# koide3/small_gicp

Measured on AMD Instinct MI355X. Metric: GICP iterations/sec (1M<->1M pts), higher is better.
Workload: dtype f32; 1 GPU; C3: GICP, per-point covariances k=20, 1000000 target <-> 1000000 source points, max_corr_dist 1.0 m; parallelism=single GPU

## Files before the change

include/small_gicp_amd_debug.h:

```cpp
#ifndef SMALL_GICP_AMD_DEBUG_H
#define SMALL_GICP_AMD_DEBUG_H

#include "small_gicp_amd.h"

#ifdef __cplusplus
extern "C" {
#endif

int sga_problem_set_search_stats(sga_context* ctx, sga_problem* pb, int enabled);
int sga_problem_get_search_stats(sga_context* ctx, const sga_problem* pb, int* leaves_per_point);
int sga_problem_get_sorted_points(sga_context* ctx, const sga_problem* pb, float* xyzw);
int sga_problem_get_last_plan(const sga_problem* pb, int out[8]);
int sga_problem_get_grid_stats(const sga_problem* pb, uint64_t out[6]);
void sga_set_grid_mode(int mode, long long min_points);
void sga_set_knn_wave_max(long long max_points);
int sga_index_spacing(const sga_index* index, double* spacing);
int sga_debug_kd_tree(sga_context* ctx, const sga_index* index, int* depth, float* nodes, float* xyzw);
int sga_debug_index_bbox(const sga_index* index, float lo[3], float hi[3]);
int sga_debug_forest_launches(unsigned long long* launches);
int sga_debug_voxelgrid_plan(const sga_cloud* cloud, double leaf, int out[9]);
int sga_debug_set_voxelgrid_epoch(sga_context* ctx, unsigned epoch);
int sga_debug_timer_start(sga_context* ctx);
int sga_debug_timer_stop(sga_context* ctx, double* ms);
#define SGA_FRAME_CHECK_DOUBLES 32
void sga_debug_shard_frame_pack(const double origin[3], double out[SGA_FRAME_CHECK_DOUBLES]);
int sga_debug_shard_frame_agree(const double sum[SGA_FRAME_CHECK_DOUBLES]);
int sga_debug_kd_trips(unsigned long long* out16);
int sga_debug_kd_wave_times(unsigned long long* out, int waves);

#ifdef __cplusplus
}
#endif
#endif
```

small_gicp_amd/_lib.py:

```python
import ctypes as C
import os
import sys

_HERE = os.path.dirname(os.path.abspath(__file__))
LIB_PATH = os.environ.get("SGA_LIB_PATH") or os.path.join(_HERE, "lib", "libsmall_gicp_amd.so")

SGA_OK = 0
ICP, PLANE_ICP, GICP = 0, 1, 2
FLAT_NORMALS, FLAT_COVS = 1, 2
ROBUST_NONE, ROBUST_HUBER, ROBUST_CAUCHY = 0, 1, 2
LEVENBERG_MARQUARDT, GAUSS_NEWTON = 0, 1
MATH_FP32, MATH_FP64 = 0, 1
ACCUM_DOUBLES = 30


class SgaError(RuntimeError):
    pass


class FactorParams(C.Structure):
    _fields_ = [("factor_kind", C.c_int), ("robust_kind", C.c_int), ("robust_c", C.c_double), ("max_dist_sq", C.c_double), ("math_mode", C.c_int)]


class RegistrationSettingC(C.Structure):
# ... 121 lines not shown
    ("sga_problem_get_sorted_points", C.c_int, [C.c_void_p, C.c_void_p, C.c_void_p]),
    ("sga_problem_get_grid_stats", C.c_int, [C.c_void_p, C.POINTER(C.c_uint64)]),
    ("sga_problem_get_last_plan", C.c_int, [C.c_void_p, C.POINTER(C.c_int)]),
    ("sga_set_grid_mode", None, [C.c_int, C.c_longlong]),
    ("sga_host_alloc", C.c_int, [C.c_size_t, C.POINTER(C.c_void_p)]),
    ("sga_host_free", C.c_int, [C.c_void_p]),
    ("sga_index_spacing", C.c_int, [C.c_void_p, C.POINTER(C.c_double)]),
    ("sga_set_knn_wave_max", None, [C.c_longlong]),
    ("sga_debug_kd_tree", C.c_int, [C.c_void_p, C.c_void_p, C.POINTER(C.c_int), C.c_void_p, C.c_void_p]),
    ("sga_debug_voxelgrid_plan", C.c_int, [C.c_void_p, C.c_double, C.POINTER(C.c_int)]),
    ("sga_debug_set_voxelgrid_epoch", C.c_int, [C.c_void_p, C.c_uint]),
    ("sga_debug_timer_start", C.c_int, [C.c_void_p]),
    ("sga_debug_timer_stop", C.c_int, [C.c_void_p, C.POINTER(C.c_double)]),
    ("sga_debug_shard_frame_pack", None, [C.POINTER(C.c_double), C.POINTER(C.c_double)]),
    ("sga_debug_shard_frame_agree", C.c_int, [C.POINTER(C.c_double)]),
    ("sga_debug_kd_trips", C.c_int, [C.c_void_p]),
    ("sga_debug_kd_wave_times", C.c_int, [C.c_void_p, C.c_int]),
    ("sga_set_search_mode", None, [C.c_int, C.c_int, C.c_int]),
    ("sga_get_warm_limit", C.c_double, []),
    ("sga_problem_get_pass_stats", C.c_int, [_vp, _vp, C.POINTER(C.c_uint64), C.POINTER(C.c_uint64), C.POINTER(C.c_uint64)]),
    ("sga_registration_setting_default", None, [C.POINTER(RegistrationSettingC)]),
    ("sga_align", C.c_int, [_vp, _vp, _vp, _dp, C.POINTER(RegistrationSettingC), C.POINTER(ResultC)]),
    ("sga_align_problem", C.c_int, [_vp, _vp, _dp, C.POINTER(RegistrationSettingC), C.POINTER(ResultC)]),
    ("sga_multi_create", C.c_int, [C.POINTER(C.c_int), C.c_int, _pvp]),
    ("sga_multi_destroy", C.c_int, [_vp]),
    ("sga_multi_num_devices", C.c_int, [_vp]),
    ("sga_multi_set_target_f64", C.c_int, [_vp, _dp, _dp, _dp, C.c_size_t]),
    ("sga_multi_set_target_f32", C.c_int, [_vp, _fp, _fp, _fp, C.c_size_t]),
    ("sga_multi_set_source_f32", C.c_int, [_vp, _fp, _fp, _fp, C.c_size_t, _dp]),
    ("sga_multi_set_target_f32_origin", C.c_int, [_vp, _fp, _fp, _fp, C.c_size_t, _dp]),
# ... 46 lines not shown
```

small_gicp_amd/api.py:

```python
import ctypes as C

import numpy as np

from . import _lib
from ._lib import GICP, ICP, PLANE_ICP, FactorParams, RegistrationSettingC, ResultC, check, load

_FACTOR_BY_NAME = {"ICP": ICP, "PLANE_ICP": PLANE_ICP, "GICP": GICP, "VGICP": GICP}


def _fp(a):
    return None if a is None else a.ctypes.data_as(C.POINTER(C.c_float))


def _dp(a):
    return None if a is None else a.ctypes.data_as(C.POINTER(C.c_double))


def _T16(T):
    T = np.eye(4) if T is None else np.asarray(T, dtype=np.float64).reshape(4, 4)
    return np.ascontiguousarray(T.T).reshape(16)


class Context:

# ... 759 lines not shown
        return RegistrationResult(res)

    def search_stats(self, enable=None):
        if enable is not None:
            check(load().sga_problem_set_search_stats(self.ctx.h, self.h, 1 if enable else 0))
            return None
        out = np.zeros(len(self.source), dtype=np.int32)
        check(load().sga_problem_get_search_stats(self.ctx.h, self.h, out.ctypes.data_as(C.c_void_p)))
        return out

    def sorted_points(self):
        out = np.zeros((len(self.source), 4), dtype=np.float32)
        check(load().sga_problem_get_sorted_points(self.ctx.h, self.h, out.ctypes.data_as(C.c_void_p)))
        return out

    def pass_stats(self):
        c, w, f = C.c_uint64(), C.c_uint64(), C.c_uint64()
        check(load().sga_problem_get_pass_stats(self.ctx.h, self.h, C.byref(c), C.byref(w), C.byref(f)))
        g = (C.c_uint64 * 6)()
        check(load().sga_problem_get_grid_stats(self.h, g))
        return {"cold_passes": c.value, "warm_passes": w.value, "walked_points": f.value, "grid_passes": g[0], "grid_open": g[1], "grid_rings": g[2], "grid_cell_m": g[3] * 1e-6,
                "adj_queries": g[4], "adj_unsettled": g[5]}


def _T16s(Ts, count):
    if Ts is None:
        Ts = [None] * count
    if len(Ts) != count:
        raise ValueError(f"{len(Ts)} poses for {count} pairs")
    return np.ascontiguousarray(np.stack([_T16(T) for T in Ts]).reshape(count, 16)) if count else np.zeros((0, 16))


class BatchProblem:

    def __init__(self, problems):
        self.problems = list(problems)
        self.ctx = self.problems[0].ctx if self.problems else default_context()
# ... 333 lines not shown
```

small_gicp_amd/csrc/common.hpp:

```cpp
#pragma once
#include <hip/hip_runtime.h>

#include <atomic>
#include <cstdarg>
#include <cstdint>
#include <cstdio>
#include <cstdlib>
#include <cstring>
#include <string>
#include <vector>

#include "../../include/small_gicp_amd.h"
#include "../../include/small_gicp_amd_debug.h"

namespace sga {

void set_error(const char* fmt, ...);
int fail(int code, const char* fmt, ...);

#define SGA_HIP(expr)                                                                                             \
  do {                                                                                                            \
    hipError_t _e = (expr);                                                                                       \
    if (_e != hipSuccess) return ::sga::fail(SGA_ERR_HIP, "%s:%d %s -> %s", __FILE__, __LINE__, #expr, hipGetErrorString(_e)); \
  } while (0)
// ... 219 lines not shown
  bool frame_checked = false;
  bool has_normals = false, has_covs = false;
  sga::DevBuf<float4> pts;
  sga::DevBuf<sga::Cov8> cov;
  const float4* pts_view = nullptr;
  const sga::Cov8* cov_view = nullptr;
  const float4* src_pts() const { return pts_view ? pts_view : pts.p; }
  const sga::Cov8* src_cov() const { return cov_view ? cov_view : cov.p; }
  sga::DevBuf<int> corr;
  sga::DevBuf<int> hint;
  sga::DevBuf<int> hint2;
  sga::DevBuf<float> rex;
  sga::DevBuf<int> dbg_leaves;
  sga::DevBuf<uint32_t> walked;
  bool state_fresh = false;
  double T_prev[16] = {0};
  bool prev_valid = false;
  int prev_math = 0;
  int lin_factor = -1;
  double lin_T[16] = {0};
  bool maha_valid = false;
  int last_math = 0;
  float bbox_lo[3] = {0, 0, 0}, bbox_hi[3] = {0, 0, 0};
  uint64_t cold_passes = 0, warm_passes = 0;
  uint64_t grid_passes = 0;
  sga::DevBuf<uint32_t> grid_stats;
  bool grid_stats_pending = false;
  uint64_t grid_open_total = 0, grid_ring_total = 0;
  double grid_open_frac = 0.0;
  sga::DevBuf<uint32_t> tile_cost, tile_order;
// ... 15 lines not shown
```

small_gicp_amd/csrc/linearize.hip:

```cpp
#include <algorithm>
#include <chrono>
#include <thread>
#include <type_traits>
#include <utility>

#include "batch.hpp"
#include "common.hpp"
#include "device_math.hpp"
#include "uniform.hpp"
#include "cell_grid.hpp"
#include "kd_search.hpp"
#include "projective.hpp"
#include "voxel_hash.hpp"

void sga_profile_collect_pending(sga_context* ctx);

namespace sga {

int comm_allreduce_sum(sga_context* ctx, double* d_buf, size_t count);
template <typename Real>
int grid_search_pass(sga_context* ctx, const sga_index* idx, const float4* src_pts, int n, const Rigid<Real>& T, float reach2, int* nn, int* nn2, float* rex, uint32_t* stats);
int grid_rings_for(const sga_index* idx, double reach);

#ifndef SGA_SPACING_REF
// ... 126 lines not shown

template <typename Real>
struct NNParams {
  const float4* __restrict__ src_pts;
  int n;
  KdView kd;
  Rigid<Real> T;
  float bound2;
  float within2;
  float slack_min, slack_max;
  float cert_pad;
  int* __restrict__ nn;
  int* __restrict__ nn2;
  float* __restrict__ rex;
  int check;
  Rigid<Real> T_prev;
  uint32_t* __restrict__ walked;
  const uint32_t* __restrict__ tile_order;
  uint32_t* __restrict__ tile_cost;
  int* __restrict__ leaves;
  double inv_leaf;
  int chunk_tiles;
  int fast;
  GridView grid;
  int grid_walk;
};

__device__ __forceinline__ float certify(float rex, float moved, bool has_neighbour, float d2_new, float within2, float pad) {
  const float lim = rex - moved * 1.000001f;
  const float lim_d = lim - moved * pad;
// ... 9 lines not shown
  if (!exact) {
    const KdBestFast f = kd_nearest_fast<BLOCK>(p.kd, fx, fy, fz, p.bound2, seed, kd_stack, tid, slack);
    nb = f.best;
    exact = f.ambiguous;
  }
  if (exact) nb = kd_nearest<BLOCK>(p.kd, fx, fy, fz, p.bound2, seed, kd_stack, tid, slack);
  p.nn[i] = nb.idx;
  p.nn2[i] = nb.idx2;
  p.rex[i] = rex_from_r2(nb.r2);
  if (p.leaves != nullptr) p.leaves[i] = nb.leaves;
  return nb.idx;
}

template <typename Real, int BLOCK, bool CHECK>
__device__ __forceinline__ int search_lane(const NNParams<Real>& p, int tile, int i, const float4& ps, float fx, float fy, float fz, uint32_t* __restrict__ kd_stack) {
  int seed = p.nn[i];
  float slack = 0.f;
  if constexpr (CHECK) {
    Real ox, oy, oz;
    transform_point<Real>(p.T_prev, ps.x, ps.y, ps.z, ox, oy, oz);
    const float moved = sqrtf(kd_dist2(static_cast<float>(ox), static_cast<float>(oy), static_cast<float>(oz), fx, fy, fz));
    const int cand2 = p.nn2[i];
    float d1 = INFINITY, d2 = INFINITY;
    if (seed >= 0) {
      const float4 c = p.kd.pts[seed];
      d1 = kd_dist2(c.x, c.y, c.z, fx, fy, fz);
    }
    if (cand2 >= 0) {
      const float4 c = p.kd.pts[cand2];
      d2 = kd_dist2(c.x, c.y, c.z, fx, fy, fz);
    }
// ... 98 lines not shown
  uint32_t node = 1;
  int depth = 0, sp = 0;
  KdState s = kd_state(p.bound2, 0.f);

  for (;;) {
    while (tile < tile_end && q_count <= kQueueCap - 64) {
      const int i = tile * 64 + lane;
      bool need = i < p.n;
      float fx = 0.f, fy = 0.f, fz = 0.f, slack = 0.f;
      int seed = -1, cand2 = -1;
      if (need) {
        const float4 ps = p.src_pts[i];
        Real x, y, z;
        transform_point<Real>(p.T, ps.x, ps.y, ps.z, x, y, z);
        fx = static_cast<float>(x), fy = static_cast<float>(y), fz = static_cast<float>(z);
        seed = p.nn[i];
        cand2 = p.nn2[i];
        if constexpr (CHECK) {
          Real ox, oy, oz;
          transform_point<Real>(p.T_prev, ps.x, ps.y, ps.z, ox, oy, oz);
          const float moved = sqrtf(kd_dist2(static_cast<float>(ox), static_cast<float>(oy), static_cast<float>(oz), fx, fy, fz));
          float d1 = INFINITY, d2 = INFINITY;
          if (seed >= 0) {
            const float4 c = p.kd.pts[seed];
            d1 = kd_dist2(c.x, c.y, c.z, fx, fy, fz);
          }
          if (cand2 >= 0) {
            const float4 c = p.kd.pts[cand2];
            d2 = kd_dist2(c.x, c.y, c.z, fx, fy, fz);
          }
          const bool swap = cand2 >= 0 && (d2 < d1 || (d2 == d1 && cand2 < seed));
          const int best = swap ? cand2 : seed;
// ... 876 lines not shown
    acc += wave_sum_f64(static_cast<double>(e));
  }
  if (lane == 0) sh_e[wave] = acc;
  __syncthreads();
  if (threadIdx.x == 0) {
    double s = 0.0;
    for (int w = 0; w < kTile / 64; w++) s += sh_e[w];
    if (p.tail.enabled)
      __hip_atomic_store(&p.partials[blockIdx.x], s, __ATOMIC_RELAXED, __HIP_MEMORY_SCOPE_AGENT);
    else
      p.partials[blockIdx.x] = s;
  }
  if (p.tail.enabled) fused_tail(p.tail, p.partials, gridDim.x, 1, 1);
}

constexpr int kReduceGroups = 64;

constexpr int kReduceSlices = 8;
__global__ __launch_bounds__(kReduceSlices * kCols) void reduce_rows_kernel(
  const double* __restrict__ partials, int nrows, int ncols, int row_stride, double* __restrict__ stage, unsigned* __restrict__ ticket, double* __restrict__ out, int out_n, double* __restrict__ host,
  unsigned long long seq, int derive, const uint32_t* __restrict__ stats) {
  __shared__ double sh[kReduceSlices][kCols];
  __shared__ unsigned sh_ticket;
  const int c = threadIdx.x & (kCols - 1), s = threadIdx.x / kCols;
  const int G = gridDim.x;
  double a0 = 0.0, a1 = 0.0, a2 = 0.0, a3 = 0.0;
  if (c < ncols) {
    const int step = G * kReduceSlices;
    int r = blockIdx.x + G * s;
    for (; r + 3 * step < nrows; r += 4 * step) {
      const double v0 = partials[static_cast<size_t>(r) * row_stride + c], v1 = partials[static_cast<size_t>(r + step) * row_stride + c];
      const double v2 = partials[static_cast<size_t>(r + 2 * step) * row_stride + c], v3 = partials[static_cast<size_t>(r + 3 * step) * row_stride + c];
      a0 += v0, a1 += v1, a2 += v2, a3 += v3;
    }
    for (; r < nrows; r += step) a0 += partials[static_cast<size_t>(r) * row_stride + c];
  }
  sh[s][c] = (a0 + a1) + (a2 + a3);
  __syncthreads();
  auto fold = [&]() {
    if (threadIdx.x < kCols) {
      double t = 0.0;
#pragma unroll
      for (int k = 0; k < kReduceSlices; k++) t += sh[k][threadIdx.x];
      sh[0][threadIdx.x] = t;
    }
    __syncthreads();
  };
  fold();
  if (G > 1) {
    if (threadIdx.x < kCols) __hip_atomic_store(&stage[blockIdx.x * kCols + threadIdx.x], sh[0][threadIdx.x], __ATOMIC_RELAXED, __HIP_MEMORY_SCOPE_AGENT);
    asm volatile("s_waitcnt vmcnt(0)" ::: "memory");
    __syncthreads();
// ... 27 lines not shown
  if (G > 1 && threadIdx.x == 0) __hip_atomic_store(ticket, 0u, __ATOMIC_RELAXED, __HIP_MEMORY_SCOPE_AGENT);
  if (host != nullptr) {
    __threadfence_system();
    __syncthreads();
    if (threadIdx.x == 0) __hip_atomic_store(reinterpret_cast<unsigned long long*>(host + kSeqWord), seq, __ATOMIC_RELEASE, __HIP_MEMORY_SCOPE_SYSTEM);
  }
}

__global__ __launch_bounds__(kReduceSlices * kCols) void batch_reduce_rows_kernel(const BatchPair* __restrict__ pairs, unsigned* __restrict__ ticket, double* __restrict__ host, double* __restrict__ seq_word, unsigned long long seq) {
  __shared__ double sh[kReduceSlices][kCols];
  __shared__ unsigned sh_ticket;
  const BatchPair* d = uniform_const(pairs + blockIdx.x);
  const double* __restrict__ partials = d->p.partials;
  const int nrows = d->ntiles, out_row = d->pair;
  const int c = threadIdx.x & (kCols - 1), s = threadIdx.x / kCols;
  double a0 = 0.0, a1 = 0.0, a2 = 0.0, a3 = 0.0;
  if (c < kModelCols) {
    constexpr int step = kReduceSlices;
    int r = s;
    for (; r + 3 * step < nrows; r += 4 * step) {
      const double v0 = partials[static_cast<size_t>(r) * kRow + c], v1 = partials[static_cast<size_t>(r + step) * kRow + c];
      const double v2 = partials[static_cast<size_t>(r + 2 * step) * kRow + c], v3 = partials[static_cast<size_t>(r + 3 * step) * kRow + c];
      a0 += v0, a1 += v1, a2 += v2, a3 += v3;
    }
    for (; r < nrows; r += step) a0 += partials[static_cast<size_t>(r) * kRow + c];
  }
  sh[s][c] = (a0 + a1) + (a2 + a3);
  __syncthreads();
  if (threadIdx.x < kCols) {
    double t = 0.0;
#pragma unroll
    for (int k = 0; k < kReduceSlices; k++) t += sh[k][threadIdx.x];
    sh[0][threadIdx.x] = t;
  }
  __syncthreads();
  if (threadIdx.x < kRow) {
    const int cc = threadIdx.x;
    const double t = is_derived_col(cc) ? derived_entry(cc, sh[0]) : sh[0][cc];
    host[static_cast<size_t>(out_row) * kRow + cc] = cc < kModelCols ? t : 0.0;
  }
  __threadfence_system();
  __syncthreads();
  if (threadIdx.x == 0) sh_ticket = __hip_atomic_fetch_add(ticket, 1u, __ATOMIC_ACQ_REL, __HIP_MEMORY_SCOPE_AGENT);
  __syncthreads();
  if (sh_ticket != gridDim.x - 1) return;
  if (threadIdx.x == 0) {
    __hip_atomic_store(ticket, 0u, __ATOMIC_RELAXED, __HIP_MEMORY_SCOPE_AGENT);
    __threadfence_system();
    __hip_atomic_store(reinterpret_cast<unsigned long long*>(seq_word), seq, __ATOMIC_RELEASE, __HIP_MEMORY_SCOPE_SYSTEM);
  }
}

__global__ __launch_bounds__(1024) void tile_order_kernel(const uint32_t* __restrict__ cost, uint32_t* __restrict__ order, int num_tiles) {
  __shared__ uint32_t hist[64], start[64];
  const int per_xcd = num_tiles >> 3;
  const int x = blockIdx.x, first = x * per_xcd;
  if (threadIdx.x < 64) hist[threadIdx.x] = 0u;
  __syncthreads();
  for (int k = threadIdx.x; k < per_xcd; k += blockDim.x) atomicAdd(&hist[63u - min(63u, cost[first + k] >> 8)], 1u);
  __syncthreads();
  if (threadIdx.x == 0) {
    uint32_t acc = 0u;
    for (int b = 0; b < 64; b++) {
      start[b] = acc;
      acc += hist[b];
    }
  }
  __syncthreads();
  for (int k = threadIdx.x; k < per_xcd; k += blockDim.x) {
    const uint32_t pos = atomicAdd(&start[63u - min(63u, cost[first + k] >> 8)], 1u);
    order[first + pos] = static_cast<uint32_t>(first + k);
  }
  if (x == 0)
    for (int t = 8 * per_xcd + threadIdx.x; t < num_tiles; t += blockDim.x) order[t] = static_cast<uint32_t>(t);
}

static size_t partial_rows(size_t n) { return std::max<size_t>(kMaxBlocks, (n + 63) / 64); }

static int reduce_groups(int nrows) { return nrows > 256 ? std::min(kReduceGroups, std::max(8, nrows / 128)) : 1; }

static void launch_reduce(sga_context* ctx, const double* partials, int nrows, int ncols, int row_stride, double* stage, double* out, int out_n, double* host, unsigned long long seq, bool derive = false, const uint32_t* stats = nullptr) {
  const int groups = reduce_groups(nrows);
  hipLaunchKernelGGL(reduce_rows_kernel, dim3(groups), dim3(kReduceSlices * kCols), 0, ctx->stream, partials, nrows, ncols, row_stride, stage, ctx->d_ticket.p, out, out_n, host, seq, derive ? 1 : 0, stats);
}

template <typename T>
static T env_or(const char* name, T d) {
  const char* s = getenv(name);
  return s == nullptr ? d : std::is_floating_point_v<T> ? static_cast<T>(atof(s)) : static_cast<T>(atoll(s));
}

constexpr int kLinPts = 4;
constexpr int kLinPtsMin = 750000;
constexpr int kLinPtsMinF64 = 131072;

static double g_warm_delta = env_or("SGA_WARM_DELTA", 0.1);

static int g_search_queue = env_or("SGA_SEARCH_QUEUE", 2);
// ... 231 lines not shown
  q.kd = p.kd;
  q.T = p.T;
  q.within2 = p.bound2;
  q.slack_min = static_cast<float>(kSlackMin * unit), q.slack_max = static_cast<float>(kSlackMax * unit);
  q.cert_pad = std::max(g_cert_pad, 0.f);
  q.bound2 = p.bound2 * (1.f + kSearchMargin) * (1.f + kSearchMargin);
  q.nn = pb->hint.p, q.nn2 = pb->hint2.p, q.rex = pb->rex.p, q.walked = pb->walked.p;
  q.fast = g_fast_scan;
  q.leaves = pb->dbg_leaves.n >= pb->n ? pb->dbg_leaves.p : nullptr;

  const PassPlan plan = plan_pass<Real>(ctx, pb, q, displacement, unit, host_rejector);
  p.num_tiles = factor_tiles(p.n, plan.pts);
  const int blocks = grid_blocks(p.num_tiles);
  p.tail = FusedTail{plan.tail ? 1 : 0, ctx->d_ticket.p, d_out30, out_n, host, seq};
  q.check = plan.warm ? 1 : 0;
  if (plan.warm) q.T_prev = rigid_from_colmajor<Real>(pb->T_prev);
  if (plan.grid) {
    q.grid_walk = g_grid_walk;
    q.grid = make_grid_view(idx);
  }
  q.chunk_tiles = plan.chunk_tiles;

  const bool timed = ctx->profiling && (ctx->lin_seq++ % ctx->profile_period) == 0;
  if (timed) {
    sga_profile_collect_pending(ctx);
    (void)hipEventRecord(ctx->ev0, ctx->stream);
    ctx->pending_warm = plan.warm;
  }
  int rows = p.n > 0 ? blocks : 0;
  const bool first_pass = !pb->prev_valid;
  if (!voxel) pb->prev_valid = false;
  pb->state_fresh = false;
  if (plan.route != Route::kFactors) {
    if (q.leaves != nullptr) SGA_HIP(hipMemsetAsync(q.leaves, 0, pb->n * sizeof(int), ctx->stream));
    if (plan.grid && (first_pass || (plan.route != Route::kGrid && !plan.warm))) pb->grid_open_frac = 0.0;
    pb->order_tiles = 0;
    const size_t words = static_cast<size_t>(p.kd.depth);
    const dim3 sgrid((p.n + kSearchBlock - 1) / kSearchBlock), sblock(kSearchBlock);
    switch (plan.route) {
      case Route::kGrid:
        if (pb->grid_stats.n < 4) {
          SGA_TRY(pb->grid_stats.alloc(4));
          SGA_HIP(hipMemsetAsync(pb->grid_stats.p, 0, 4 * sizeof(uint32_t), ctx->stream));
        }
        SGA_TRY(grid_search_pass<Real>(ctx, idx, pb->src_pts(), p.n, p.T, q.bound2, pb->hint.p, pb->hint2.p, pb->rex.p, pb->grid_stats.p));
        pb->grid_passes++;
        break;
      case Route::kCertify:
        if constexpr (sizeof(Real) == 4) {
          p.cert_nn = q.nn, p.cert_nn2 = q.nn2, p.cert_rex = q.rex, p.cert_walked = q.walked;
          p.T_prev = q.T_prev, p.cert_within2 = q.within2, p.cert_pad = q.cert_pad;
          p.cert_slack_min = q.slack_min, p.cert_slack_max = q.slack_max;
          const size_t lds = std::max<size_t>(words, 1) * 64 * sizeof(uint32_t) * (kTile / 64);
          with_factor(fp->factor_kind, [&](auto f) { hipLaunchKernelGGL((certify_linearize_kernel<Real, decltype(f)::value, 1>), dim3(blocks), dim3(kTile), lds, ctx->stream, p, q); });
        }
        break;
      case Route::kFusedLane:
        if constexpr (sizeof(Real) == 4) {
// ... 68 lines not shown
    }
  }
  if (p.n > 0 && !plan.fused()) {
    with_factor(fp->factor_kind, [&](auto f) {
      constexpr int F = decltype(f)::value;
      if (flat)
        launch_linearize<Real, F, 2>(ctx->stream, p, blocks, plan.pts);
      else if (proj) {
        hipLaunchKernelGGL((projective_linearize_kernel<Real, F, 1>), dim3(blocks), dim3(kTile), 0, ctx->stream, p, make_proj_view(idx));
      } else if (voxel) {
        if constexpr (F != SGA_PLANE_ICP) launch_linearize<Real, F, 1>(ctx->stream, p, blocks, plan.pts);
      } else
        launch_linearize<Real, F, 0>(ctx->stream, p, blocks, plan.pts);
    });
  }
  if (!plan.tail) launch_reduce(ctx, pb->partials.p, rows, ncols, kRow, pb->partials.p + partial_rows(pb->n) * kRow, d_out30, out_n, host, seq, true, plan.route == Route::kGrid ? pb->grid_stats.p : nullptr);
  pb->grid_stats_pending = plan.route == Route::kGrid && !plan.tail && out_n > kStatsCol + 1;
  {
    const int lp[8] = {static_cast<int>(plan.route), plan.warm, plan.grid, plan.pts, plan.tail, plan.chunk_tiles, plan.tail ? 0 : rows, plan.tail ? 0 : reduce_groups(rows)};
    std::copy(lp, lp + 8, pb->last_plan);
  }
  if (timed) {
    (void)hipEventRecord(ctx->ev1, ctx->stream);
    ctx->pending |= 1;
  }
  if (plan.order_record) {
    hipLaunchKernelGGL(tile_order_kernel, dim3(8), dim3(1024), 0, ctx->stream, pb->tile_cost.p, pb->tile_order.p, rows);
    pb->order_tiles = static_cast<unsigned>(rows);
    pb->order_stream = ctx->stream;
  }
  SGA_HIP(hipGetLastError());
  pb->last_math = math;
  pb->lin_factor = fp->factor_kind;
  memcpy(pb->lin_T, T, sizeof(pb->lin_T));
  pb->maha_valid = p.store_maha != 0;
  if (!voxel) {
    memcpy(pb->T_prev, T, sizeof(pb->T_prev));
    pb->prev_valid = true;
    pb->prev_math = math;
    if (plan.warm)
      pb->warm_passes++;
    else
      pb->cold_passes++;
  }
  return SGA_OK;
}

template <typename Real>
__global__ void recompute_maha_kernel(const Cov8* __restrict__ src_cov, const Cov8* __restrict__ tgt_cov, const int* __restrict__ corr, int n, Rigid<Real> T, Real* __restrict__ maha) {
  const int i = blockIdx.x * blockDim.x + threadIdx.x;
  if (i >= n) return;
  const int j = corr[i];
  if (j < 0) return;
  const Sym3<Real> Cs = load_sym<Real>(src_cov, i);
// ... 418 lines not shown
    const double* Tp = problem_pose(pb, T + 16 * k, Td);
    if (Tp != Td) memcpy(Td, Tp, 16 * sizeof(double));
    BatchPair d{};
    d.p = factor_params<float>(pb, fp, Td, false);
    d.p.kd = make_kd_view(idx);
    d.p.partials = pb->partials.p;
    d.q.src_pts = pb->src_pts();
    d.q.n = d.p.n;
    d.q.kd = d.p.kd;
    d.q.T = d.p.T;
    d.q.within2 = d.p.bound2;
    d.q.bound2 = d.p.bound2 * (1.f + kSearchMargin) * (1.f + kSearchMargin);
    d.q.nn = pb->hint.p, d.q.nn2 = pb->hint2.p, d.q.rex = pb->rex.p, d.q.walked = pb->walked.p;
    d.q.fast = g_fast_scan;
    d.ntiles = bt->tiles[k];
    d.seedless = seedless ? 1 : 0;
    d.pair = k;
    prefix[a] = blocks;
    blocks += (d.ntiles + 7) / 8 * 8;
    pairs[a] = d;
  }
  prefix[order.size()] = blocks;
  const int nactive = static_cast<int>(order.size());
  const unsigned long long seq = ++bt->seq;
  SGA_HIP(hipMemcpyAsync(bt->d_round.p, bt->h_round, batch_round_bytes(count), hipMemcpyHostToDevice, ctx->stream));
  const int* d_prefix = reinterpret_cast<const int*>(bt->d_round.p);
  const BatchPair* d_pairs = reinterpret_cast<const BatchPair*>(bt->d_round.p + batch_pairs_offset(count));
  for (int k : order) {
    sga_problem* pb = bt->problems[k];
    pb->prev_valid = false;
    pb->model_valid = false;
// ... 11 lines not shown
  if (rc != SGA_OK) {
    (void)hipMemsetAsync(bt->ticket.p, 0, sizeof(unsigned), ctx->stream);
    return rc;
  }
  for (size_t a = 0; a < order.size(); a++) {
    const int k = order[a];
    sga_problem* pb = bt->problems[k];
    const double* Td = &Tdev[16 * a];
    pb->last_math = SGA_MATH_FP32;
    pb->lin_factor = fp->factor_kind;
    memcpy(pb->lin_T, Td, sizeof(pb->lin_T));
    pb->maha_valid = false;
    memcpy(pb->T_prev, Td, sizeof(pb->T_prev));
    pb->prev_valid = true;
    pb->prev_math = SGA_MATH_FP32;
    pb->cold_passes++;
    pb->grid_stats_pending = false;
    const int lp[8] = {static_cast<int>(Route::kFusedLane), 0, 0, 1, 0, 0, bt->tiles[k], 1};
    std::copy(lp, lp + 8, pb->last_plan);
    memcpy(pb->model, bt->h_out + static_cast<size_t>(k) * kRow, sizeof(pb->model));
    memcpy(pb->model_T, Td, sizeof(pb->model_T));
    pb->model_valid = true;
  }
  return SGA_OK;
}
}

extern "C" {

int sga_linearize(sga_context* ctx, sga_problem* pb, const sga_factor_params* fp, const double T[16], double H[36], double b[6], double* e, uint64_t* num_inliers) {
// ... 101 lines not shown
  if (enabled) return pb->dbg_leaves.alloc(pb->n);
  pb->dbg_leaves.release();
  return SGA_OK;
}
int sga_problem_get_sorted_points(sga_context* ctx, const sga_problem* pb, float* xyzw) {
  if (!ctx || !pb || !xyzw) return fail(SGA_ERR_INVALID, "null argument");
  if (pb->n == 0) return SGA_OK;
  SGA_ENTER(ctx);
  SGA_HIP(hipMemcpyAsync(xyzw, pb->src_pts(), pb->n * sizeof(float4), hipMemcpyDeviceToHost, ctx->stream));
  SGA_HIP(hipStreamSynchronize(ctx->stream));
  return SGA_OK;
}
int sga_problem_get_last_plan(const sga_problem* pb, int out[8]) {
  if (!pb || !out) return fail(SGA_ERR_INVALID, "null argument");
  std::copy(pb->last_plan, pb->last_plan + 8, out);
  return SGA_OK;
}
int sga_problem_get_search_stats(sga_context* ctx, const sga_problem* pb, int* leaves_per_point) {
  if (!ctx || !pb || !leaves_per_point) return fail(SGA_ERR_INVALID, "null argument");
  if (pb->dbg_leaves.n < pb->n) return fail(SGA_ERR_INVALID, "search statistics are not enabled");
  SGA_ENTER(ctx);
  SGA_HIP(hipMemcpyAsync(leaves_per_point, pb->dbg_leaves.p, pb->n * sizeof(int), hipMemcpyDeviceToHost, ctx->stream));
  SGA_HIP(hipStreamSynchronize(ctx->stream));
  return SGA_OK;
}

#ifdef SGA_KD_TRIPS
int sga_debug_kd_trips(unsigned long long* out16) {
  unsigned long long zero[16] = {0};
  if (hipMemcpyFromSymbol(out16, HIP_SYMBOL(g_kd_trips), sizeof(zero)) != hipSuccess) return SGA_ERR_HIP;
// ... 19 lines not shown
#define SGA_PRELOAD_FACTOR(F)                                        \
  SGA_PRELOAD(search_linearize_kernel<float, F, false>);            \
  SGA_PRELOAD(search_linearize_kernel<float, F, true>);             \
  SGA_PRELOAD(nn_search_queue_kernel<float, true, F>);              \
  SGA_PRELOAD(certify_linearize_kernel<float, F, 1>);               \
  SGA_PRELOAD(linearize_kernel<float, F, 0, kLinPts>);              \
  SGA_PRELOAD(linearize_kernel<float, F, 0, 1>);                   \
  SGA_PRELOAD(batch_search_linearize_kernel<F>)
  SGA_PRELOAD_FACTOR(SGA_GICP);
  SGA_PRELOAD_FACTOR(SGA_PLANE_ICP);
  SGA_PRELOAD_FACTOR(SGA_ICP);
  SGA_PRELOAD(linearize_kernel<float, SGA_GICP, 1, kLinPts>);
  SGA_PRELOAD(linearize_kernel<float, SGA_GICP, 1, 1>);
  SGA_PRELOAD(reduce_rows_kernel);
  SGA_PRELOAD(batch_reduce_rows_kernel);
  SGA_PRELOAD(tile_order_kernel);
  SGA_PRELOAD(publish_kernel);
  SGA_PRELOAD(error_kernel<float, SGA_GICP>);
#undef SGA_PRELOAD_FACTOR
#undef SGA_PRELOAD
  (void)hipGetLastError();
}
}

extern "C" {

void sga_set_grid_mode(int mode, long long min_points) {
  if (mode >= 0) sga::g_grid_mode = mode;
  if (min_points >= 0) sga::g_grid_min_points = min_points;
}

// ... 8 lines not shown
```

small_gicp_amd/csrc/optimizer.hip:

```cpp
#include <cmath>
#include <cstdio>

#include "batch.hpp"
#include "common.hpp"

namespace sga {

struct M4 {
  double a[16];
};

static M4 mul(const M4& A, const M4& B) {
  M4 C;
  for (int c = 0; c < 4; c++)
    for (int r = 0; r < 4; r++) {
      double s = 0;
      for (int k = 0; k < 4; k++) s += A.a[4 * k + r] * B.a[4 * c + k];
      C.a[4 * c + r] = s;
    }
  return C;
}

static M4 se3_exp(const double d[6]) {
  const double wx = d[0], wy = d[1], wz = d[2];
// ... 352 lines not shown
  const M4 m = se3_exp(twist);
  memcpy(T, m.a, sizeof(m.a));
}

int sga_optimize(const sga_registration_setting* setting, const double init_T[16], sga_linearize_fn linearize, sga_error_fn error, void* user, sga_result* out) {
  if (!setting || !init_T || !linearize || !out) return fail(SGA_ERR_INVALID, "null argument");
  if (setting->optimizer == SGA_LEVENBERG_MARQUARDT && !error) return fail(SGA_ERR_INVALID, "LM needs an error callback");
  return optimize_impl(*setting, init_T, linearize, error, user, out);
}

int sga_align_problem(sga_context* ctx, sga_problem* problem, const double init_T[16], const sga_registration_setting* setting, sga_result* out) {
  if (!ctx || !problem || !setting || !out) return fail(SGA_ERR_INVALID, "null argument");
  static const double I16[16] = {1, 0, 0, 0, 0, 1, 0, 0, 0, 0, 1, 0, 0, 0, 0, 1};
  if (problem->target->n <= 10) std::fprintf(stderr, "warning: target point cloud is too small. |target|=%zu\n", problem->target->n);
  if (problem->n <= 10) std::fprintf(stderr, "warning: source point cloud is too small. |source|=%zu\n", problem->n);
  if (!problem->state_fresh) {
    SGA_HIP(hipSetDevice(ctx->device));
    if (problem->n > 0) SGA_HIP(hipMemsetAsync(problem->hint.p, 0xff, problem->n * sizeof(int), ctx->stream));
    if (problem->n > 0 && problem->hint2.n >= problem->n) SGA_HIP(hipMemsetAsync(problem->hint2.p, 0xff, problem->n * sizeof(int), ctx->stream));
  }
  problem->prev_valid = false;
  GpuReduction g{ctx, problem, &setting->factor};
  return optimize_impl(*setting, init_T ? init_T : I16, gpu_linearize, gpu_error, &g, out);
}

int sga_optimize_batch(const sga_registration_setting* setting, size_t count, const double* init_T, sga_batch_linearize_fn linearize, sga_batch_error_fn error, void* user, sga_result* out) {
  if (!setting || !linearize) return fail(SGA_ERR_INVALID, "null argument");
  if (setting->optimizer == SGA_LEVENBERG_MARQUARDT && !error) return fail(SGA_ERR_INVALID, "LM needs an error callback");
  if (count == 0) return SGA_OK;
  if (!out) return fail(SGA_ERR_INVALID, "null argument");
  return optimize_batch_impl(*setting, count, init_T, linearize, error, user, out);
}

int sga_align_batch(sga_context* ctx, sga_batch* batch, const double* init_T, const sga_registration_setting* setting, sga_result* out) {
  if (!setting) return fail(SGA_ERR_INVALID, "null argument");
// ... 25 lines not shown
```

Measured before the change: 8908 iterations/s.

## Fold tile-order sort into reduce kernel and replace hint memsets with seedless flag

The separate tile_order_kernel launch is removed and its work is done by eight extra blocks appended to the reduce_rows grid. The per-align hipMemsetAsync calls that reset the nn/nn2 hint arrays are replaced by a hints_void flag, which makes the first cold pass ignore the stale seeds. Both changes cut kernel/memset launches per pass and per align, at the cost of a more complex reduce kernel and extra state tracking. Debug counters and introspection APIs are also added.

```diff
diff --git a/include/small_gicp_amd_debug.h b/include/small_gicp_amd_debug.h
--- a/include/small_gicp_amd_debug.h
+++ b/include/small_gicp_amd_debug.h
@@ -25,6 +25,10 @@
 #define SGA_FRAME_CHECK_DOUBLES 32
 void sga_debug_shard_frame_pack(const double origin[3], double out[SGA_FRAME_CHECK_DOUBLES]);
 int sga_debug_shard_frame_agree(const double sum[SGA_FRAME_CHECK_DOUBLES]);
+int sga_debug_reduce_rows(sga_context* ctx, const double* rows, int nrows, int derive, int groups, int kind, double out[96]);
+int sga_problem_get_search_state(sga_context* ctx, const sga_problem* pb, int* nn, int* nn2, float* rex);
+int sga_problem_get_tile_order(sga_context* ctx, const sga_problem* pb, unsigned* cost, unsigned* order, size_t capacity, size_t* tiles);
+int sga_debug_pass_launches(unsigned long long out[3]);
 int sga_debug_kd_trips(unsigned long long* out16);
 int sga_debug_kd_wave_times(unsigned long long* out, int waves);
 
diff --git a/small_gicp_amd/_lib.py b/small_gicp_amd/_lib.py
--- a/small_gicp_amd/_lib.py
+++ b/small_gicp_amd/_lib.py
@@ -159,6 +159,10 @@
     ("sga_debug_timer_stop", C.c_int, [C.c_void_p, C.POINTER(C.c_double)]),
     ("sga_debug_shard_frame_pack", None, [C.POINTER(C.c_double), C.POINTER(C.c_double)]),
     ("sga_debug_shard_frame_agree", C.c_int, [C.POINTER(C.c_double)]),
+    ("sga_debug_reduce_rows", C.c_int, [C.c_void_p, C.c_void_p, C.c_int, C.c_int, C.c_int, C.c_int, C.POINTER(C.c_double)]),
+    ("sga_problem_get_search_state", C.c_int, [C.c_void_p, C.c_void_p, C.c_void_p, C.c_void_p, C.c_void_p]),
+    ("sga_problem_get_tile_order", C.c_int, [C.c_void_p, C.c_void_p, C.c_void_p, C.c_void_p, C.c_size_t, C.POINTER(C.c_size_t)]),
+    ("sga_debug_pass_launches", C.c_int, [C.POINTER(C.c_ulonglong)]),
     ("sga_debug_kd_trips", C.c_int, [C.c_void_p]),
     ("sga_debug_kd_wave_times", C.c_int, [C.c_void_p, C.c_int]),
     ("sga_set_search_mode", None, [C.c_int, C.c_int, C.c_int]),
diff --git a/small_gicp_amd/api.py b/small_gicp_amd/api.py
--- a/small_gicp_amd/api.py
+++ b/small_gicp_amd/api.py
@@ -797,6 +797,20 @@
         check(load().sga_problem_get_sorted_points(self.ctx.h, self.h, out.ctypes.data_as(C.c_void_p)))
         return out
 
+    def search_state(self):
+        n = len(self.source)
+        nn, nn2, rex = np.zeros(n, np.int32), np.zeros(n, np.int32), np.zeros(n, np.float32)
+        check(load().sga_problem_get_search_state(self.ctx.h, self.h, nn.ctypes.data_as(C.c_void_p), nn2.ctypes.data_as(C.c_void_p), rex.ctypes.data_as(C.c_void_p)))
+        return nn, nn2, rex
+
+    def tile_order(self):
+        tiles = C.c_size_t()
+        check(load().sga_problem_get_tile_order(self.ctx.h, self.h, None, None, 0, C.byref(tiles)))
+        cost, order = np.zeros(tiles.value, np.uint32), np.zeros(tiles.value, np.uint32)
+        if tiles.value:
+            check(load().sga_problem_get_tile_order(self.ctx.h, self.h, cost.ctypes.data_as(C.c_void_p), order.ctypes.data_as(C.c_void_p), tiles.value, C.byref(tiles)))
+        return cost, order
+
     def pass_stats(self):
         c, w, f = C.c_uint64(), C.c_uint64(), C.c_uint64()
         check(load().sga_problem_get_pass_stats(self.ctx.h, self.h, C.byref(c), C.byref(w), C.byref(f)))
@@ -804,6 +818,20 @@
         check(load().sga_problem_get_grid_stats(self.h, g))
         return {"cold_passes": c.value, "warm_passes": w.value, "walked_points": f.value, "grid_passes": g[0], "grid_open": g[1], "grid_rings": g[2], "grid_cell_m": g[3] * 1e-6,
                 "adj_queries": g[4], "adj_unsettled": g[5]}
+
+
+def debug_reduce_rows(rows, derive=False, groups=0, batch=False, ctx=None):
+    rows = np.ascontiguousarray(rows, dtype=np.float64).reshape(-1, 96)
+    out = np.zeros(96)
+    c = ctx or default_context()
+    check(load().sga_debug_reduce_rows(c.h, rows.ctypes.data_as(C.c_void_p), rows.shape[0], 1 if derive else 0, int(groups), 1 if batch else 0, _dp(out)))
+    return out
+
+
+def debug_pass_launches():
+    v = (C.c_ulonglong * 3)()
+    check(load().sga_debug_pass_launches(v))
+    return {"reduce": v[0], "reduce_with_sort": v[1], "fills": v[2]}
 
 
 def _T16s(Ts, count):
diff --git a/small_gicp_amd/csrc/common.hpp b/small_gicp_amd/csrc/common.hpp
--- a/small_gicp_amd/csrc/common.hpp
+++ b/small_gicp_amd/csrc/common.hpp
@@ -257,6 +257,7 @@
   sga::DevBuf<int> dbg_leaves;
   sga::DevBuf<uint32_t> walked;
   bool state_fresh = false;
+  bool hints_void = false;
   double T_prev[16] = {0};
   bool prev_valid = false;
   int prev_math = 0;
diff --git a/small_gicp_amd/csrc/linearize.hip b/small_gicp_amd/csrc/linearize.hip
--- a/small_gicp_amd/csrc/linearize.hip
+++ b/small_gicp_amd/csrc/linearize.hip
@@ -1,4 +1,5 @@
 #include <algorithm>
+#include <atomic>
 #include <chrono>
 #include <thread>
 #include <type_traits>
@@ -164,6 +165,7 @@
   int* __restrict__ nn2;
   float* __restrict__ rex;
   int check;
+  int seedless;
   Rigid<Real> T_prev;
   uint32_t* __restrict__ walked;
   const uint32_t* __restrict__ tile_order;
@@ -203,7 +205,7 @@
 
 template <typename Real, int BLOCK, bool CHECK>
 __device__ __forceinline__ int search_lane(const NNParams<Real>& p, int tile, int i, const float4& ps, float fx, float fy, float fz, uint32_t* __restrict__ kd_stack) {
-  int seed = p.nn[i];
+  int seed = p.seedless ? -1 : p.nn[i];
   float slack = 0.f;
   if constexpr (CHECK) {
     Real ox, oy, oz;
@@ -332,8 +334,10 @@
         Real x, y, z;
         transform_point<Real>(p.T, ps.x, ps.y, ps.z, x, y, z);
         fx = static_cast<float>(x), fy = static_cast<float>(y), fz = static_cast<float>(z);
-        seed = p.nn[i];
-        cand2 = p.nn2[i];
+        if (!p.seedless) {
+          seed = p.nn[i];
+          cand2 = p.nn2[i];
+        }
         if constexpr (CHECK) {
           Real ox, oy, oz;
           transform_point<Real>(p.T_prev, ps.x, ps.y, ps.z, ox, oy, oz);
@@ -1240,28 +1244,58 @@
   if (p.tail.enabled) fused_tail(p.tail, p.partials, gridDim.x, 1, 1);
 }
 
+__device__ __forceinline__ void tile_order_share(const uint32_t* __restrict__ cost, uint32_t* __restrict__ order, int num_tiles, int x) {
+  __shared__ uint32_t hist[64], start[64];
+  const int per_xcd = num_tiles >> 3;
+  const int first = x * per_xcd;
+  if (threadIdx.x < 64) hist[threadIdx.x] = 0u;
+  __syncthreads();
+  for (int k = threadIdx.x; k < per_xcd; k += blockDim.x) atomicAdd(&hist[63u - min(63u, cost[first + k] >> 8)], 1u);
+  __syncthreads();
+  if (threadIdx.x == 0) {
+    uint32_t acc = 0u;
+    for (int b = 0; b < 64; b++) {
+      start[b] = acc;
+      acc += hist[b];
+    }
+  }
+  __syncthreads();
+  for (int k = threadIdx.x; k < per_xcd; k += blockDim.x) {
+    const uint32_t pos = atomicAdd(&start[63u - min(63u, cost[first + k] >> 8)], 1u);
+    order[first + pos] = static_cast<uint32_t>(first + k);
+  }
+  if (x == 0)
+    for (int t = 8 * per_xcd + threadIdx.x; t < num_tiles; t += blockDim.x) order[t] = static_cast<uint32_t>(t);
+}
+
 constexpr int kReduceGroups = 64;
+static std::atomic<unsigned long long> g_pass_launches[3];
 
 constexpr int kReduceSlices = 8;
+
+__device__ __forceinline__ double sum_rows_chains(const double* __restrict__ partials, int r0, int step, int nrows, int row_stride, int c) {
+  double a0 = 0.0, a1 = 0.0, a2 = 0.0, a3 = 0.0;
+  int r = r0;
+  for (; r + 3 * step < nrows; r += 4 * step) {
+    const double v0 = partials[static_cast<size_t>(r) * row_stride + c], v1 = partials[static_cast<size_t>(r + step) * row_stride + c];
+    const double v2 = partials[static_cast<size_t>(r + 2 * step) * row_stride + c], v3 = partials[static_cast<size_t>(r + 3 * step) * row_stride + c];
+    a0 += v0, a1 += v1, a2 += v2, a3 += v3;
+  }
+  for (; r < nrows; r += step) a0 += partials[static_cast<size_t>(r) * row_stride + c];
+  return (a0 + a1) + (a2 + a3);
+}
+
 __global__ __launch_bounds__(kReduceSlices * kCols) void reduce_rows_kernel(
-  const double* __restrict__ partials, int nrows, int ncols, int row_stride, double* __restrict__ stage, unsigned* __restrict__ ticket, double* __restrict__ out, int out_n, double* __restrict__ host,
-  unsigned long long seq, int derive, const uint32_t* __restrict__ stats) {
+  const double* __restrict__ partials, int nrows, int ncols, int row_stride, int G, double* __restrict__ stage, unsigned* __restrict__ ticket, double* __restrict__ out, int out_n, double* __restrict__ host,
+  unsigned long long seq, int derive, const uint32_t* __restrict__ stats, const uint32_t* __restrict__ tile_cost, uint32_t* __restrict__ tile_order, int order_tiles) {
   __shared__ double sh[kReduceSlices][kCols];
   __shared__ unsigned sh_ticket;
+  if (static_cast<int>(blockIdx.x) >= G) {
+    tile_order_share(tile_cost, tile_order, order_tiles, static_cast<int>(blockIdx.x) - G);
+    return;
+  }
   const int c = threadIdx.x & (kCols - 1), s = threadIdx.x / kCols;
-  const int G = gridDim.x;
-  double a0 = 0.0, a1 = 0.0, a2 = 0.0, a3 = 0.0;
-  if (c < ncols) {
-    const int step = G * kReduceSlices;
-    int r = blockIdx.x + G * s;
-    for (; r + 3 * step < nrows; r += 4 * step) {
-      const double v0 = partials[static_cast<size_t>(r) * row_stride + c], v1 = partials[static_cast<size_t>(r + step) * row_stride + c];
-      const double v2 = partials[static_cast<size_t>(r + 2 * step) * row_stride + c], v3 = partials[static_cast<size_t>(r + 3 * step) * row_stride + c];
-      a0 += v0, a1 += v1, a2 += v2, a3 += v3;
-    }
-    for (; r < nrows; r += step) a0 += partials[static_cast<size_t>(r) * row_stride + c];
-  }
-  sh[s][c] = (a0 + a1) + (a2 + a3);
+  sh[s][c] = c < ncols ? sum_rows_chains(partials, static_cast<int>(blockIdx.x) + G * s, G * kReduceSlices, nrows, row_stride, c) : 0.0;
   __syncthreads();
   auto fold = [&]() {
     if (threadIdx.x < kCols) {
@@ -1319,18 +1353,7 @@
   const double* __restrict__ partials = d->p.partials;
   const int nrows = d->ntiles, out_row = d->pair;
   const int c = threadIdx.x & (kCols - 1), s = threadIdx.x / kCols;
-  double a0 = 0.0, a1 = 0.0, a2 = 0.0, a3 = 0.0;
-  if (c < kModelCols) {
-    constexpr int step = kReduceSlices;
-    int r = s;
-    for (; r + 3 * step < nrows; r += 4 * step) {
-      const double v0 = partials[static_cast<size_t>(r) * kRow + c], v1 = partials[static_cast<size_t>(r + step) * kRow + c];
-      const double v2 = partials[static_cast<size_t>(r + 2 * step) * kRow + c], v3 = partials[static_cast<size_t>(r + 3 * step) * kRow + c];
-      a0 += v0, a1 += v1, a2 += v2, a3 += v3;
-    }
-    for (; r < nrows; r += step) a0 += partials[static_cast<size_t>(r) * kRow + c];
-  }
-  sh[s][c] = (a0 + a1) + (a2 + a3);
+  sh[s][c] = c < kModelCols ? sum_rows_chains(partials, s, kReduceSlices, nrows, kRow, c) : 0.0;
   __syncthreads();
   if (threadIdx.x < kCols) {
     double t = 0.0;
@@ -1356,37 +1379,18 @@
   }
 }
 
-__global__ __launch_bounds__(1024) void tile_order_kernel(const uint32_t* __restrict__ cost, uint32_t* __restrict__ order, int num_tiles) {
-  __shared__ uint32_t hist[64], start[64];
-  const int per_xcd = num_tiles >> 3;
-  const int x = blockIdx.x, first = x * per_xcd;
-  if (threadIdx.x < 64) hist[threadIdx.x] = 0u;
-  __syncthreads();
-  for (int k = threadIdx.x; k < per_xcd; k += blockDim.x) atomicAdd(&hist[63u - min(63u, cost[first + k] >> 8)], 1u);
-  __syncthreads();
-  if (threadIdx.x == 0) {
-    uint32_t acc = 0u;
-    for (int b = 0; b < 64; b++) {
-      start[b] = acc;
-      acc += hist[b];
-    }
-  }
-  __syncthreads();
-  for (int k = threadIdx.x; k < per_xcd; k += blockDim.x) {
-    const uint32_t pos = atomicAdd(&start[63u - min(63u, cost[first + k] >> 8)], 1u);
-    order[first + pos] = static_cast<uint32_t>(first + k);
-  }
-  if (x == 0)
-    for (int t = 8 * per_xcd + threadIdx.x; t < num_tiles; t += blockDim.x) order[t] = static_cast<uint32_t>(t);
-}
-
 static size_t partial_rows(size_t n) { return std::max<size_t>(kMaxBlocks, (n + 63) / 64); }
 
 static int reduce_groups(int nrows) { return nrows > 256 ? std::min(kReduceGroups, std::max(8, nrows / 128)) : 1; }
 
-static void launch_reduce(sga_context* ctx, const double* partials, int nrows, int ncols, int row_stride, double* stage, double* out, int out_n, double* host, unsigned long long seq, bool derive = false, const uint32_t* stats = nullptr) {
-  const int groups = reduce_groups(nrows);
-  hipLaunchKernelGGL(reduce_rows_kernel, dim3(groups), dim3(kReduceSlices * kCols), 0, ctx->stream, partials, nrows, ncols, row_stride, stage, ctx->d_ticket.p, out, out_n, host, seq, derive ? 1 : 0, stats);
+static void launch_reduce(sga_context* ctx, const double* partials, int nrows, int ncols, int row_stride, double* stage, double* out, int out_n, double* host, unsigned long long seq, bool derive = false, const uint32_t* stats = nullptr,
+                          const uint32_t* tile_cost = nullptr, uint32_t* tile_order = nullptr, int order_tiles = 0, int force_groups = 0) {
+  const int groups = force_groups > 0 ? force_groups : reduce_groups(nrows);
+  const int sorters = tile_order != nullptr ? 8 : 0;
+  hipLaunchKernelGGL(reduce_rows_kernel, dim3(groups + sorters), dim3(kReduceSlices * kCols), 0, ctx->stream, partials, nrows, ncols, row_stride, groups, stage, ctx->d_ticket.p, out, out_n, host, seq, derive ? 1 : 0, stats, tile_cost,
+                     tile_order, order_tiles);
+  g_pass_launches[0].fetch_add(1, std::memory_order_relaxed);
+  if (sorters != 0) g_pass_launches[1].fetch_add(1, std::memory_order_relaxed);
 }
 
 template <typename T>
@@ -1648,6 +1652,7 @@
   const int blocks = grid_blocks(p.num_tiles);
   p.tail = FusedTail{plan.tail ? 1 : 0, ctx->d_ticket.p, d_out30, out_n, host, seq};
   q.check = plan.warm ? 1 : 0;
+  q.seedless = pb->hints_void && !plan.warm ? 1 : 0;
   if (plan.warm) q.T_prev = rigid_from_colmajor<Real>(pb->T_prev);
   if (plan.grid) {
     q.grid_walk = g_grid_walk;
@@ -1666,7 +1671,10 @@
   if (!voxel) pb->prev_valid = false;
   pb->state_fresh = false;
   if (plan.route != Route::kFactors) {
-    if (q.leaves != nullptr) SGA_HIP(hipMemsetAsync(q.leaves, 0, pb->n * sizeof(int), ctx->stream));
+    if (q.leaves != nullptr) {
+      SGA_HIP(hipMemsetAsync(q.leaves, 0, pb->n * sizeof(int), ctx->stream));
+      g_pass_launches[2].fetch_add(1, std::memory_order_relaxed);
+    }
     if (plan.grid && (first_pass || (plan.route != Route::kGrid && !plan.warm))) pb->grid_open_frac = 0.0;
     pb->order_tiles = 0;
     const size_t words = static_cast<size_t>(p.kd.depth);
@@ -1676,6 +1684,7 @@
         if (pb->grid_stats.n < 4) {
           SGA_TRY(pb->grid_stats.alloc(4));
           SGA_HIP(hipMemsetAsync(pb->grid_stats.p, 0, 4 * sizeof(uint32_t), ctx->stream));
+          g_pass_launches[2].fetch_add(1, std::memory_order_relaxed);
         }
         SGA_TRY(grid_search_pass<Real>(ctx, idx, pb->src_pts(), p.n, p.T, q.bound2, pb->hint.p, pb->hint2.p, pb->rex.p, pb->grid_stats.p));
         pb->grid_passes++;
@@ -1774,7 +1783,9 @@
         launch_linearize<Real, F, 0>(ctx->stream, p, blocks, plan.pts);
     });
   }
-  if (!plan.tail) launch_reduce(ctx, pb->partials.p, rows, ncols, kRow, pb->partials.p + partial_rows(pb->n) * kRow, d_out30, out_n, host, seq, true, plan.route == Route::kGrid ? pb->grid_stats.p : nullptr);
+  if (!plan.tail)
+    launch_reduce(ctx, pb->partials.p, rows, ncols, kRow, pb->partials.p + partial_rows(pb->n) * kRow, d_out30, out_n, host, seq, true, plan.route == Route::kGrid ? pb->grid_stats.p : nullptr,
+                  plan.order_record ? pb->tile_cost.p : nullptr, plan.order_record ? pb->tile_order.p : nullptr, rows);
   pb->grid_stats_pending = plan.route == Route::kGrid && !plan.tail && out_n > kStatsCol + 1;
   {
     const int lp[8] = {static_cast<int>(plan.route), plan.warm, plan.grid, plan.pts, plan.tail, plan.chunk_tiles, plan.tail ? 0 : rows, plan.tail ? 0 : reduce_groups(rows)};
@@ -1785,7 +1796,6 @@
     ctx->pending |= 1;
   }
   if (plan.order_record) {
-    hipLaunchKernelGGL(tile_order_kernel, dim3(8), dim3(1024), 0, ctx->stream, pb->tile_cost.p, pb->tile_order.p, rows);
     pb->order_tiles = static_cast<unsigned>(rows);
     pb->order_stream = ctx->stream;
   }
@@ -1798,6 +1808,7 @@
     memcpy(pb->T_prev, T, sizeof(pb->T_prev));
     pb->prev_valid = true;
     pb->prev_math = math;
+    if (plan.route != Route::kFactors) pb->hints_void = false;
     if (plan.warm)
       pb->warm_passes++;
     else
@@ -2246,7 +2257,7 @@
     d.q.nn = pb->hint.p, d.q.nn2 = pb->hint2.p, d.q.rex = pb->rex.p, d.q.walked = pb->walked.p;
     d.q.fast = g_fast_scan;
     d.ntiles = bt->tiles[k];
-    d.seedless = seedless ? 1 : 0;
+    d.seedless = seedless || pb->hints_void ? 1 : 0;
     d.pair = k;
     prefix[a] = blocks;
     blocks += (d.ntiles + 7) / 8 * 8;
@@ -2288,6 +2299,7 @@
     memcpy(pb->T_prev, Td, sizeof(pb->T_prev));
     pb->prev_valid = true;
     pb->prev_math = SGA_MATH_FP32;
+    if (bt->tiles[k] > 0) pb->hints_void = false;
     pb->cold_passes++;
     pb->grid_stats_pending = false;
     const int lp[8] = {static_cast<int>(Route::kFusedLane), 0, 0, 1, 0, 0, bt->tiles[k], 1};
@@ -2419,6 +2431,62 @@
 int sga_problem_get_last_plan(const sga_problem* pb, int out[8]) {
   if (!pb || !out) return fail(SGA_ERR_INVALID, "null argument");
   std::copy(pb->last_plan, pb->last_plan + 8, out);
+  return SGA_OK;
+}
+int sga_debug_reduce_rows(sga_context* ctx, const double* rows, int nrows, int derive, int groups, int kind, double out[96]) {
+  if (!ctx || !out || nrows < 0 || (nrows > 0 && !rows) || groups < 0 || groups > kReduceGroups || kind < 0 || kind > 1) return fail(SGA_ERR_INVALID, "invalid argument");
+  SGA_ENTER(ctx);
+  const size_t nr = static_cast<size_t>(nrows);
+  DevBuf<double> buf, res;
+  DevBuf<unsigned> ticket;
+  SGA_TRY(buf.alloc(std::max<size_t>(nr, 1) * kRow + static_cast<size_t>(kReduceGroups) * kCols));
+  SGA_TRY(res.alloc(kRow + 1));
+  if (nrows > 0) SGA_HIP(hipMemcpyAsync(buf.p, rows, nr * kRow * sizeof(double), hipMemcpyHostToDevice, ctx->stream));
+  if (kind == 0) {
+    launch_reduce(ctx, buf.p, nrows, kModelCols, kRow, buf.p + std::max<size_t>(nr, 1) * kRow, res.p, kRow, nullptr, 0, derive != 0, nullptr, nullptr, nullptr, 0, groups);
+  } else {
+    DevBuf<BatchPair> pair;
+    SGA_TRY(pair.alloc(1));
+    SGA_TRY(ticket.alloc(1));
+    BatchPair d{};
+    d.p.partials = buf.p;
+    d.ntiles = nrows;
+    d.pair = 0;
+    SGA_HIP(hipMemcpyAsync(pair.p, &d, sizeof(d), hipMemcpyHostToDevice, ctx->stream));
+    SGA_HIP(hipMemsetAsync(ticket.p, 0, sizeof(unsigned), ctx->stream));
+    hipLaunchKernelGGL(batch_reduce_rows_kernel, dim3(1), dim3(kReduceSlices * kCols), 0, ctx->stream, pair.p, ticket.p, res.p, res.p + kRow, 1ull);
+    SGA_HIP(hipGetLastError());
+    SGA_HIP(hipStreamSynchronize(ctx->stream));
+  }
+  SGA_HIP(hipGetLastError());
+  SGA_HIP(hipMemcpyAsync(out, res.p, kRow * sizeof(double), hipMemcpyDeviceToHost, ctx->stream));
+  SGA_HIP(hipStreamSynchronize(ctx->stream));
+  return SGA_OK;
+}
+int sga_problem_get_search_state(sga_context* ctx, const sga_problem* pb, int* nn, int* nn2, float* rex) {
+  if (!ctx || !pb) return fail(SGA_ERR_INVALID, "null argument");
+  if (pb->n == 0) return SGA_OK;
+  SGA_ENTER(ctx);
+  if (nn != nullptr) SGA_HIP(hipMemcpyAsync(nn, pb->hint.p, pb->n * sizeof(int), hipMemcpyDeviceToHost, ctx->stream));
+  if (nn2 != nullptr) SGA_HIP(hipMemcpyAsync(nn2, pb->hint2.p, pb->n * sizeof(int), hipMemcpyDeviceToHost, ctx->stream));
+  if (rex != nullptr) SGA_HIP(hipMemcpyAsync(rex, pb->rex.p, pb->n * sizeof(float), hipMemcpyDeviceToHost, ctx->stream));
+  SGA_HIP(hipStreamSynchronize(ctx->stream));
+  return SGA_OK;
+}
+int sga_problem_get_tile_order(sga_context* ctx, const sga_problem* pb, unsigned* cost, unsigned* order, size_t capacity, size_t* tiles) {
+  if (!ctx || !pb || !tiles) return fail(SGA_ERR_INVALID, "null argument");
+  *tiles = pb->order_tiles;
+  if (pb->order_tiles == 0 || cost == nullptr || order == nullptr) return SGA_OK;
+  if (capacity < pb->order_tiles) return fail(SGA_ERR_INVALID, "room for %zu tiles, the pass recorded %u", capacity, pb->order_tiles);
+  SGA_ENTER(ctx);
+  SGA_HIP(hipMemcpyAsync(cost, pb->tile_cost.p, pb->order_tiles * sizeof(unsigned), hipMemcpyDeviceToHost, ctx->stream));
+  SGA_HIP(hipMemcpyAsync(order, pb->tile_order.p, pb->order_tiles * sizeof(unsigned), hipMemcpyDeviceToHost, ctx->stream));
+  SGA_HIP(hipStreamSynchronize(ctx->stream));
+  return SGA_OK;
+}
+int sga_debug_pass_launches(unsigned long long out[3]) {
+  if (!out) return fail(SGA_ERR_INVALID, "null argument");
+  for (int k = 0; k < 3; k++) out[k] = g_pass_launches[k].load(std::memory_order_relaxed);
   return SGA_OK;
 }
 int sga_problem_get_search_stats(sga_context* ctx, const sga_problem* pb, int* leaves_per_point) {
@@ -2468,7 +2536,6 @@
   SGA_PRELOAD(linearize_kernel<float, SGA_GICP, 1, 1>);
   SGA_PRELOAD(reduce_rows_kernel);
   SGA_PRELOAD(batch_reduce_rows_kernel);
-  SGA_PRELOAD(tile_order_kernel);
   SGA_PRELOAD(publish_kernel);
   SGA_PRELOAD(error_kernel<float, SGA_GICP>);
 #undef SGA_PRELOAD_FACTOR
diff --git a/small_gicp_amd/csrc/optimizer.hip b/small_gicp_amd/csrc/optimizer.hip
--- a/small_gicp_amd/csrc/optimizer.hip
+++ b/small_gicp_amd/csrc/optimizer.hip
@@ -390,11 +390,7 @@
   static const double I16[16] = {1, 0, 0, 0, 0, 1, 0, 0, 0, 0, 1, 0, 0, 0, 0, 1};
   if (problem->target->n <= 10) std::fprintf(stderr, "warning: target point cloud is too small. |target|=%zu\n", problem->target->n);
   if (problem->n <= 10) std::fprintf(stderr, "warning: source point cloud is too small. |source|=%zu\n", problem->n);
-  if (!problem->state_fresh) {
-    SGA_HIP(hipSetDevice(ctx->device));
-    if (problem->n > 0) SGA_HIP(hipMemsetAsync(problem->hint.p, 0xff, problem->n * sizeof(int), ctx->stream));
-    if (problem->n > 0 && problem->hint2.n >= problem->n) SGA_HIP(hipMemsetAsync(problem->hint2.p, 0xff, problem->n * sizeof(int), ctx->stream));
-  }
+  problem->hints_void = true;
   problem->prev_valid = false;
   GpuReduction g{ctx, problem, &setting->factor};
   return optimize_impl(*setting, init_T ? init_T : I16, gpu_linearize, gpu_error, &g, out);
```

New measurement: 8993 iterations/s, median of 6. About the same (+0.9%).
